# yoyololicon/spectrogram-inversion

Hardware: AMD Instinct MI355X
Metric: Griffin-Lim iterations*frames/sec at n_fft=2048 hop=512 (higher is better)
Workload: dtype f32; 1 GPU; C2: griffin_lim B64/GPU n_fft=2048 hop=512 T=1024 it=100 alpha=0.3 hann center reflect tol=0 eva_iter=10; global_batch=64, parallelism=batch-sharded x1, RCCL gather, step=phase_init + ISTFT + iterations + gather, kernel=k_fused4_td

## Files before the change

### spectrogram_inversion_amd/csrc/kernels_fast_td.h

```cpp
#pragma once
#include "fast_core.h"

namespace specinv {
namespace fast {


template <bool FIRST, typename A, typename B>
__device__ __forceinline__ const auto& td_pick(const A& a, const B& b) {
  if constexpr (FIRST) return a;
  else return b;
}


template <int R, int OV>
__device__ __forceinline__ void td_load_block(const float* __restrict__ xrow, const float* __restrict__ tailrow, long long L,
                                              int T, int c, int t_begin, int t_end, int j, int lane, int pad_mode,
                                              v2f (&q)[R / OV]) {
  if constexpr (OV == 4) load_block4<R>(xrow, tailrow, L, T, c, t_begin, t_end, j, lane, pad_mode, q);
  else load_block<R, OV>(xrow, tailrow, L, T, c, t_begin, t_end, j, lane, pad_mode, q);
}

template <int R, int OV, bool EARLY, bool EVAL>
__device__ __forceinline__ void fused_td_body(const FastArgs& a) {
  using G = Geo<R>;
  using O = Ovl<R, OV>;
  constexpr int H = G::H, M = G::M, QU = O::QU, HOP = O::HOP, NB = O::NB, PB = O::PB;
  extern __shared__ __attribute__((aligned(16))) char smem[];
  v2f* lds_win = reinterpret_cast<v2f*>(smem);
  v2f* lds_wins = lds_win + M;
  v2f* lds_tw1 = lds_win + 2 * M;
  const int wib = __builtin_amdgcn_readfirstlane(threadIdx.x >> 6);
  v2f* tr = lds_tw1 + (R - 1) * 64 + wib * G::TR;

  for (int i = threadIdx.x; i < M; i += blockDim.x) {
    const v2f wv = v2f{a.window[2 * i], a.window[2 * i + 1]};
    lds_win[i] = wv;
    lds_wins[i] = wv * a.inv_scale;
  }
  for (int i = threadIdx.x; i < (R - 1) * 64; i += blockDim.x) {
    const int k1 = i / 64 + 1, l = i & 63;
    lds_tw1[i] = unit(2.0f * (float)((l * k1) % M) / (float)M);
  }
  __syncthreads();

  int w = __builtin_amdgcn_readfirstlane(blockIdx.x * (blockDim.x >> 6) + wib);
  if (a.skew == 0 && w >= a.n_waves) return;
  const LaneConst<R> k = lane_consts<R>();
  const int lane = k.lane;
  const unsigned ulane = (unsigned)lane;
  int b = w / a.nchunks, c = w - b * a.nchunks;
  if (a.skew >= 0x10000) {
    const int cg = 3 * ((int)blockIdx.x * 4 + (wib & 3)) + (wib >> 2);
    b = cg / a.nchunks;
    c = cg - b * a.nchunks;
    w = cg;
  } else if (a.skew != 0 && (blockDim.x >> 6) == 8) {
    const int cg = 2 * ((int)blockIdx.x * 4 + (wib & 3)) + (wib >> 2);
    b = cg / a.nchunks;
    c = cg - b * a.nchunks;
    w = cg;
  } else if (a.skew != 0) {
    const int half = a.n_waves >> 1, second = w >= half ? 1 : 0, wl = w - second * half, pairs = a.nchunks >> 1;
    b = wl / pairs;
    c = 2 * (wl - b * pairs) + second;
    w = b * a.nchunks + c;
  }
  if (a.skew != 0 && w >= a.n_waves) return;
  const int t_begin = chunk_begin(c, a.T, a.nchunks, a.skew);
  const int t_end = chunk_begin(c + 1, a.T, a.nchunks, a.skew);
  const float* zrow = a.x_in + (long long)b * a.L;
  const float* tailrow = a.xtail_in + (long long)b * a.nchunks * NB * HOP;
  float* zorow = a.x_out + (long long)b * a.L;
  const bool write_x = a.x2_out != nullptr;
  float* xorow = a.x2_out + (long long)b * a.L;
  const float half_scale = 0.5f * a.fwd_scale;
  const float tds_raw = a.tds / half_scale;
  const float nlr = -a.coef;

  v2f acc[NB * QU];
#pragma unroll
  for (int i = 0; i < NB * QU; ++i) acc[i] = v2f{0.0f, 0.0f};
  double sd = 0.0, so = 0.0;
  constexpr bool TWLDS = EVAL && R >= 16;
  TwRegs<TWLDS ? 2 : R> twr_regs;
  if (!TWLDS) {
#pragma unroll
    for (int k1 = 1; k1 < R; ++k1) twr_regs.w[(TWLDS ? 1 : k1) - 1] = lds_tw1[(k1 - 1) * 64 + lane];
  }
  const TwLds twr_lds{lds_tw1, lane};
  const auto& twr = td_pick<TWLDS>(twr_lds, twr_regs);

  v2f xq[NB][QU], xn[QU];
#pragma unroll
  for (int q = 0; q < NB; ++q)
    td_load_block<R, OV>(zrow, tailrow, a.L, a.T, c, t_begin, t_end, t_begin + q, lane, a.pad_mode, xq[q]);
  td_load_block<R, OV>(zrow, tailrow, a.L, a.T, c, t_begin, t_end, t_begin + NB, lane, a.pad_mode, xn);

  constexpr bool ENVREG = !EVAL;
  v2f envc[ENVREG ? QU : 1];
  v2f envr[ENVREG ? QU : 1];
  if (ENVREG) {
    const v2f* e0 = reinterpret_cast<const v2f*>(a.env + (long long)(NB - PB) * HOP);
#pragma unroll
    for (int i = 0; i < QU; ++i) {
      envc[i] = e0[64u * i + ulane];
      envr[i] = env_rcp(envc[i]);
    }
  }
  constexpr bool WKREG = !EVAL;
  v2f wkr[WKREG ? H : 1];
  if (WKREG) {
#pragma unroll
    for (int j = 0; j < H; ++j) wkr[j] = pair_twiddle<R>(k.wn, j);
  }
  for (int t = t_begin; t < t_end; ++t) {
    asm volatile("" ::: "memory");
    v2f wn = k.wn;
    asm volatile("" : "+v"(wn));
    const long long fi = (long long)b * a.T + t;
    v4f mm[H / 2];
    v4f pp[EARLY ? H : 1];
    v2f pmid = v2f{0.0f, 0.0f};
    float mmid = 0.0f;
    __builtin_amdgcn_s_setprio(1);
    {
      const v4f* min_ = a.m_pairs + fi * (H / 2 * 64);
#pragma unroll
      for (int j = 0; j < H / 2; ++j) mm[j] = ld_stream(&min_[j * 64u + ulane]);
      if (lane == 0) {
        mmid = a.m_mid[fi];
        if (EARLY) pmid = a.Pmid_in[fi];
      }
    }
#define SPECINV_TD_C0_LOADS()                                                              \
    if (EARLY) {                                                                           \
      const v4f* pin_ = a.P_in + fi * (H * 64);                                            \
      _Pragma("unroll") for (int j = 0; j < H; ++j) pp[j] = ld_stream(&pin_[j * 64u + ulane]); \
    }
    if (!EVAL) SPECINV_TD_C0_LOADS();

    v2f z[R];
    if (EVAL) {
      const float* xrow = a.x2_in + (long long)b * a.L;
#pragma unroll
      for (int qq = 0; qq < OV; ++qq) {
        v2f q[QU];
        td_load_block<R, OV>(xrow, tailrow, a.L, a.T, c, t_begin, t_end, t + qq, lane, a.pad_mode, q);
#pragma unroll
        for (int i = 0; i < QU; ++i) z[qq * QU + i] = q[i] * lds_win[64 * (qq * QU + i) + lane];
      }
      fft_forward_t<R>(z, k, twr, tr);
      v2f rc[H];
#pragma unroll
      for (int m = H; m < R; ++m) {
        const v2f got = shfl2(z[m], k.partner);
        const v2f own = z[(m + 1) % R];
        rc[m - H] = v2f{lane == 0 ? own.x : got.x, lane == 0 ? own.y : got.y};
      }
      float fd = 0.0f, fo = 0.0f;
#pragma unroll
      for (int j = 0; j < H; ++j) {
        const v2f wk = pair_twiddle<R>(wn, j);
        v2f xk, xm;
        td_split<R>(z[j], rc[R - 1 - j - H], wk, half_scale, xk, xm);
        const float mk = (j & 1) ? mm[j / 2].z : mm[j / 2].x;
        const float mq = (j & 1) ? mm[j / 2].w : mm[j / 2].y;
        const float ok = fast_abs(xk), om = fast_abs(xm);
        const float dk = ok - mk, dm = om - mq;
        fd = fmaf(dk, dk, fmaf(dm, dm, fd));
        fo = fmaf(ok, ok, fmaf(om, om, fo));
      }
      if (lane == 0) {
        const float o = fast_abs(z[H] * v2f{a.fwd_scale, -a.fwd_scale});
        const float d = o - mmid;
        fd = fmaf(d, d, fd);
        fo = fmaf(o, o, fo);
      }
      sd += (double)fd;
      so += (double)fo;
      asm volatile("" ::: "memory");
      __builtin_amdgcn_sched_barrier(0);
      SPECINV_TD_C0_LOADS();
    }
#undef SPECINV_TD_C0_LOADS

    v2f zold[QU];
#pragma unroll
    for (int i = 0; i < QU; ++i) {
      zold[i] = xq[0][i];
#pragma unroll
      for (int q = 0; q < NB; ++q) z[q * QU + i] = xq[q][i] * lds_win[64 * (q * QU + i) + lane];
      z[NB * QU + i] = xn[i] * lds_win[64 * (NB * QU + i) + lane];
#pragma unroll
      for (int q = 0; q + 1 < NB; ++q) xq[q][i] = xq[q + 1][i];
      xq[NB - 1][i] = xn[i];
    }
    if (t + 1 < t_end)
      td_load_block<R, OV>(zrow, tailrow, a.L, a.T, c, t_begin, t_end, t + OV, lane, a.pad_mode, xn);
    __builtin_amdgcn_s_setprio(0);

    fft_forward_t<R>(z, k, twr, tr);

    v2f rc[H];
#pragma unroll
    for (int m = H; m < R; ++m) {
      const v2f got = shfl2(z[m], k.partner);
      const v2f own = z[(m + 1) % R];
      rc[m - H] = v2f{lane == 0 ? own.x : got.x, lane == 0 ? own.y : got.y};
    }

    v2f back[H];
    {
      v2f sk[H], sm[H], tt[H], yy[H], hh[H];
#pragma unroll
      for (int j = 0; j < H; ++j) {
        const v2f wk = WKREG ? wkr[WKREG ? j : 0] : pair_twiddle<R>(wn, j);
        td_split_raw<R>(z[j], rc[R - 1 - j - H], wk, sk[j], sm[j]);
        if (EARLY) {
          sk[j] = __builtin_elementwise_fma(v2f{pp[j].x, pp[j].y}, v2f{tds_raw, tds_raw}, sk[j]);
          sm[j] = __builtin_elementwise_fma(v2f{pp[j].z, pp[j].w}, v2f{tds_raw, tds_raw}, sm[j]);
        }
        tt[j] = v2f{ref_norm2(sk[j], 4.0f * kRefFloor), ref_norm2(sm[j], 4.0f * kRefFloor)};
      }
#pragma unroll
      for (int j = 0; j < H; ++j) yy[j] = v2f{__builtin_amdgcn_rsqf(tt[j].x), __builtin_amdgcn_rsqf(tt[j].y)};
#pragma unroll
      for (int j = 0; j < H; ++j) hh[j] = tt[j] * yy[j];
#pragma unroll
      for (int j = 0; j < H; ++j) tt[j] = __builtin_elementwise_fma(-hh[j], yy[j], v2f{1.0f, 1.0f});
#pragma unroll
      for (int j = 0; j < H; ++j) yy[j] = __builtin_elementwise_fma(yy[j] * 0.5f, tt[j], yy[j]);
#pragma unroll
      for (int j = 0; j < H; ++j) {
        const v2f mp = (j & 1) ? v2f{mm[j / 2].z, mm[j / 2].w} : v2f{mm[j / 2].x, mm[j / 2].y};
        sk[j] = scale_lo(sk[j], mp);
        sm[j] = scale_hi(sm[j], mp);
      }
#pragma unroll
      for (int j = 0; j < H; ++j) {
        const v2f wk = WKREG ? wkr[WKREG ? j : 0] : pair_twiddle<R>(wn, j);
        v2f ak = scale_lo(sk[j], yy[j]);
        v2f am = scale_hi(sm[j], yy[j]);
        if (j == 0 && lane == 0) {
          ak.y = 0.0f;
          am.y = 0.0f;
        }
        const v2f e2i = add_conj(ak, am);
        const v2f o2i = cmulc(sub_conj(ak, am), wk);
        z[j] = add_i(e2i, o2i);
        back[j] = conj_sub_i(e2i, o2i);
      }
    }
    v2f zmid;
    {
      v2f smid = z[H] * v2f{a.fwd_scale, -a.fwd_scale};
      if (EARLY) smid = v2f{fmaf(a.tds, pmid.x, smid.x), fmaf(a.tds, pmid.y, smid.y)};
      const v2f am = (smid * mmid) * ref_rcp_abs(ref_norm2(smid));
      zmid = am * v2f{2.0f, -2.0f};
    }
#pragma unroll
    for (int m = H; m < R; ++m) {
      const v2f got = shfl2(back[R - 1 - m], k.partner);
      const v2f l0 = (m == H) ? zmid : back[(R - m) % H];
      z[m] = v2f{lane == 0 ? l0.x : got.x, lane == 0 ? l0.y : got.y};
    }

    fft_inverse_t<R>(z, k, twr, tr);

#pragma unroll
    for (int u = 0; u < R; ++u) z[u] = z[u] * lds_wins[64 * u + lane];
    if (t >= PB) {
      const long long o0 = (long long)(t - PB) * HOP;
      const v2f* envp = reinterpret_cast<const v2f*>(a.env + o0);
      v2f* xo = reinterpret_cast<v2f*>(xorow + o0);
      v2f* zo = reinterpret_cast<v2f*>(zorow + o0);
      v2f ev[QU], er[QU];
      if (!ENVREG) {
#pragma unroll
        for (int i = 0; i < QU; ++i) {
          ev[i] = envp[64u * i + ulane];
          er[i] = env_rcp(ev[i]);
        }
      } else if (t >= NB) {
#pragma unroll
        for (int i = 0; i < QU; ++i) {
          ev[i] = envc[ENVREG ? i : 0];
          er[i] = envr[ENVREG ? i : 0];
        }
      } else {
#pragma unroll
        for (int i = 0; i < QU; ++i) ev[i] = envp[64u * i + ulane];
#pragma unroll
        for (int i = 0; i < QU; ++i) asm volatile("" : "+v"(ev[i]));
#pragma unroll
        for (int i = 0; i < QU; ++i) er[i] = env_rcp(ev[i]);
      }
#pragma unroll
      for (int i = 0; i < QU; ++i) {
        const v2f xv = env_apply_r(acc[i] + z[i], ev[i], er[i]);
        const v2f zv = v2f{fmaf(nlr, zold[i].x, xv.x), fmaf(nlr, zold[i].y, xv.y)};
        if (write_x) xo[64u * i + ulane] = xv;
        zo[64u * i + ulane] = zv;
      }
    }
#pragma unroll
    for (int i = 0; i < QU; ++i) {
#pragma unroll
      for (int q = 0; q + 1 < NB; ++q) acc[q * QU + i] = acc[(q + 1) * QU + i] + z[(q + 1) * QU + i];
      acc[(NB - 1) * QU + i] = z[NB * QU + i];
    }
  }
  if (t_end == a.T) {
#pragma unroll
    for (int q = 0; q < PB - 1; ++q) {
      const long long o0 = (long long)(a.T + q - PB) * HOP;
      const v2f* envp = reinterpret_cast<const v2f*>(a.env + o0);
      v2f* xo = reinterpret_cast<v2f*>(xorow + o0);
      v2f* zo = reinterpret_cast<v2f*>(zorow + o0);
#pragma unroll
      for (int i = 0; i < QU; ++i) {
        const v2f xv = env_apply(acc[q * QU + i], envp[64u * i + ulane]);
        if (write_x) xo[64u * i + ulane] = xv;
        zo[64u * i + ulane] = v2f{fmaf(nlr, xq[q][i].x, xv.x), fmaf(nlr, xq[q][i].y, xv.y)};
      }
    }
  } else {
    v2f* tl = reinterpret_cast<v2f*>(a.xtail_out + ((long long)b * a.nchunks + c) * NB * HOP);
#pragma unroll
    for (int q = 0; q < NB; ++q) {
      const v2f* envp = reinterpret_cast<const v2f*>(a.env + (long long)(t_end + q - PB) * HOP);
#pragma unroll
      for (int i = 0; i < QU; ++i) tl[(q * QU + i) * 64u + ulane] = env_apply(acc[q * QU + i], envp[64u * i + ulane]);
    }
  }
  if (EVAL) {
    const double d = wave_sum(sd), o = wave_sum(so);
    if (lane == 0) {
      a.partials[2 * (long long)w] = d;
      a.partials[2 * (long long)w + 1] = o;
    }
  }
}

template <int R, bool EARLY, bool EVAL>
__global__ __launch_bounds__(R == 8 ? 768 : 64 * kFused4Waves, R == 8 ? kR8Waves : kMinWaves) void k_fused4_td(FastArgs a) {
  fused_td_body<R, 4, EARLY, EVAL>(a);
}
template <int R, int OV, bool EARLY, bool EVAL>
__global__ __launch_bounds__(256, R >= 32 ? 1 : R == 8 ? kR8Waves : kMinWaves) void k_fused_td(FastArgs a) {
  fused_td_body<R, OV, EARLY, EVAL>(a);
}

constexpr int kEvalSub = kEvalPieces;
template <int R, int OV>
__global__ __launch_bounds__(256, kEvalWaves) void k_eval_td(FastArgs a) {
  using G = Geo<R>;
  using O = Ovl<R, OV>;
  constexpr int H = G::H, M = G::M, QU = O::QU, HOP = O::HOP, NB = O::NB;
  extern __shared__ __attribute__((aligned(16))) char smem[];
  v2f* lds_win = reinterpret_cast<v2f*>(smem);
  v2f* lds_tw1 = lds_win + M;
  const int wib = __builtin_amdgcn_readfirstlane(threadIdx.x >> 6);
  v2f* tr = lds_tw1 + (R - 1) * 64 + wib * G::TR;
  for (int i = threadIdx.x; i < M; i += blockDim.x) lds_win[i] = v2f{a.window[2 * i], a.window[2 * i + 1]};
  for (int i = threadIdx.x; i < (R - 1) * 64; i += blockDim.x) {
    const int k1 = i / 64 + 1, l = i & 63;
    lds_tw1[i] = unit(2.0f * (float)((l * k1) % M) / (float)M);
  }
  __syncthreads();
  const int w = __builtin_amdgcn_readfirstlane(blockIdx.x * 4 + wib);
  if (w >= a.n_waves * kEvalSub) return;
  const LaneConst<R> k = lane_consts<R>();
  const int lane = k.lane;
  const unsigned ulane = (unsigned)lane;
  const int cw = w / kEvalSub, sub = w - cw * kEvalSub;
  const int b = cw / a.nchunks, c = cw - b * a.nchunks;
  const int t_begin = chunk_begin(c, a.T, a.nchunks, a.skew), t_end = chunk_begin(c + 1, a.T, a.nchunks, a.skew);
  const int s_begin = t_begin + (sub * (t_end - t_begin)) / kEvalSub, s_end = t_begin + ((sub + 1) * (t_end - t_begin)) / kEvalSub;
  const float* xrow = a.x2_in + (long long)b * a.L;
  const float* tailrow = a.xtail_in + (long long)b * a.nchunks * NB * HOP;
  const float half_scale = 0.5f * a.fwd_scale;
  TwRegs<R> twr;
#pragma unroll
  for (int k1 = 1; k1 < R; ++k1) twr.w[k1 - 1] = lds_tw1[(k1 - 1) * 64 + lane];
  double sd = 0.0, so = 0.0;
  v2f xq[NB][QU], xn[QU];
#pragma unroll
  for (int q = 0; q < NB; ++q)
    td_load_block<R, OV>(xrow, tailrow, a.L, a.T, c, t_begin, t_end, s_begin + q, lane, a.pad_mode, xq[q]);
  td_load_block<R, OV>(xrow, tailrow, a.L, a.T, c, t_begin, t_end, s_begin + NB, lane, a.pad_mode, xn);
  for (int t = s_begin; t < s_end; ++t) {
    asm volatile("" ::: "memory");
    v2f wn = k.wn;
    asm volatile("" : "+v"(wn));
    const long long fi = (long long)b * a.T + t;
    v4f mm[H / 2];
    float mmid = 0.0f;
    {
      const v4f* min_ = a.m_pairs + fi * (H / 2 * 64);
#pragma unroll
      for (int j = 0; j < H / 2; ++j) mm[j] = ld_stream(&min_[j * 64u + ulane]);
      if (lane == 0) mmid = a.m_mid[fi];
    }
    v2f z[R];
#pragma unroll
    for (int i = 0; i < QU; ++i) {
#pragma unroll
      for (int q = 0; q < NB; ++q) z[q * QU + i] = xq[q][i] * lds_win[64 * (q * QU + i) + lane];
      z[NB * QU + i] = xn[i] * lds_win[64 * (NB * QU + i) + lane];
#pragma unroll
      for (int q = 0; q + 1 < NB; ++q) xq[q][i] = xq[q + 1][i];
      xq[NB - 1][i] = xn[i];
    }
    if (t + 1 < s_end) td_load_block<R, OV>(xrow, tailrow, a.L, a.T, c, t_begin, t_end, t + OV, lane, a.pad_mode, xn);
    fft_forward_t<R>(z, k, twr, tr);
    v2f rc[H];
#pragma unroll
    for (int m = H; m < R; ++m) {
      const v2f got = shfl2(z[m], k.partner);
      const v2f own = z[(m + 1) % R];
      rc[m - H] = v2f{lane == 0 ? own.x : got.x, lane == 0 ? own.y : got.y};
    }
    float fd = 0.0f, fo = 0.0f;
#pragma unroll
    for (int j = 0; j < H; ++j) {
      const v2f wk = pair_twiddle<R>(wn, j);
      v2f xk, xm;
      td_split<R>(z[j], rc[R - 1 - j - H], wk, half_scale, xk, xm);
      const float mk = (j & 1) ? mm[j / 2].z : mm[j / 2].x;
      const float mq = (j & 1) ? mm[j / 2].w : mm[j / 2].y;
      const float ok = fast_abs(xk), om = fast_abs(xm);
      const float dk = ok - mk, dm = om - mq;
      fd = fmaf(dk, dk, fmaf(dm, dm, fd));
      fo = fmaf(ok, ok, fmaf(om, om, fo));
    }
    if (lane == 0) {
      const float o = fast_abs(z[H] * v2f{a.fwd_scale, -a.fwd_scale});
      const float d = o - mmid;
      fd = fmaf(d, d, fd);
      fo = fmaf(o, o, fo);
    }
    sd += (double)fd;
    so += (double)fo;
  }
  const double d = wave_sum(sd), o = wave_sum(so);
  if (lane == 0) {
    a.partials[2 * (long long)w] = d;
    a.partials[2 * (long long)w + 1] = o;
  }
}

}
}
```

Before: 320.3 million iterations*frames/s.

## Add specialized radix-16 TD FFT path with LDS transpose and streamline envelope handling

Adds a hand-specialized R==16 forward/inverse FFT built from explicit DFT16 stages with constant-folded twiddles, a cross-lane DFT4, and an LDS transpose through precomputed scratch pointers. The fused and eval TD kernels now call it in place of the generic fft_forward_t/fft_inverse_t. The change also reuses the env register arrays instead of copying them, applies the window multiply only to the overlap part and defers the last block's scaling into the accumulator update, and marks xn as undefined on the last iteration to avoid keeping it live. The aim is fewer ALU and shuffle operations and less register pressure in the inner frame loop. In exchange it brings an R-specific code path and more complex LDS indexing.

```diff
diff --git a/spectrogram_inversion_amd/csrc/kernels_fast_td.h b/spectrogram_inversion_amd/csrc/kernels_fast_td.h
--- a/spectrogram_inversion_amd/csrc/kernels_fast_td.h
+++ b/spectrogram_inversion_amd/csrc/kernels_fast_td.h
@@ -18,6 +18,107 @@
                                               v2f (&q)[R / OV]) {
   if constexpr (OV == 4) load_block4<R>(xrow, tailrow, L, T, c, t_begin, t_end, j, lane, pad_mode, q);
   else load_block<R, OV>(xrow, tailrow, L, T, c, t_begin, t_end, j, lane, pad_mode, q);
+}
+
+using lds_v2f = __attribute__((address_space(3))) v2f;
+struct TdScratch {
+  volatile lds_v2f* q;
+  lds_v2f* b;
+};
+template <int R>
+__device__ __forceinline__ TdScratch td_scratch(v2f* tr, const LaneConst<R>& k) {
+  TdScratch s;
+  s.q = (volatile lds_v2f*)(tr + k.tr_q);
+  s.b = (lds_v2f*)(tr + k.tr_b);
+  asm volatile("" : "+v"(s.b));
+  return s;
+}
+
+template <bool INV>
+__device__ __forceinline__ void dft4_rot2(v2f& a0, v2f& a1, v2f& a2, v2f& a3) {
+  const v2f t0 = INV ? add_i(a0, a2) : sub_i(a0, a2);
+  const v2f t1 = INV ? sub_i(a0, a2) : add_i(a0, a2);
+  const v2f t2 = a1 + a3, d = a1 - a3;
+  a0 = t0 + t2;
+  a2 = t0 - t2;
+  a1 = INV ? add_i(t1, d) : sub_i(t1, d);
+  a3 = INV ? sub_i(t1, d) : add_i(t1, d);
+}
+template <bool INV>
+__device__ __forceinline__ void td_dft16(v2f (&a)[16]) {
+  constexpr float c1 = 0.92387953251128675613f, s1 = 0.38268343236508977173f, h = 0.70710678118654752440f;
+#pragma unroll
+  for (int n0 = 0; n0 < 4; ++n0) dft4<INV>(a[n0], a[n0 + 4], a[n0 + 8], a[n0 + 12]);
+  dirmul_x4<INV, true>(a[5], a[6], a[7], a[9], v2f{c1, -s1}, v2f{h, -h}, v2f{s1, -c1}, v2f{h, -h});
+  dirmul_x4<INV, true>(a[11], a[13], a[14], a[15], v2f{-h, -h}, v2f{s1, -c1}, v2f{-h, -h}, v2f{-c1, s1});
+  dft4<INV>(a[0], a[1], a[2], a[3]);
+  dft4<INV>(a[4], a[5], a[6], a[7]);
+  dft4_rot2<INV>(a[8], a[9], a[10], a[11]);
+  dft4<INV>(a[12], a[13], a[14], a[15]);
+  v2f o[16];
+#pragma unroll
+  for (int k0 = 0; k0 < 4; ++k0)
+#pragma unroll
+    for (int k1 = 0; k1 < 4; ++k1) o[k1 + 4 * k0] = a[k0 + 4 * k1];
+#pragma unroll
+  for (int i = 0; i < 16; ++i) a[i] = o[i];
+}
+
+template <int R, typename TW>
+__device__ __forceinline__ void td_fft_forward(v2f (&z)[R], const LaneConst<R>& k, const TW& tw, v2f* __restrict__ tr,
+                                               const TdScratch& sc) {
+  if constexpr (R == 16) {
+    td_dft16<false>(z);
+    cmul_all<R, true, false, 1>(z, tw);
+#pragma unroll
+    for (int g = 0; g < R; g += 4) xlane_dft4_in<false>(z[g], z[g + 1], z[g + 2], z[g + 3]);
+#pragma unroll
+    for (int g = 0; g < R; g += 4) {
+      z[g + 2] = cmul(z[g + 2], k.postq[0]);
+      z[g + 1] = cmul(z[g + 1], k.postq[1]);
+      z[g + 3] = cmul(z[g + 3], k.postq[2]);
+    }
+#pragma unroll
+    for (int g = 0; g < R; g += 4) {
+      sc.q[(0 * R + g) * (R + 1)] = z[g];
+      sc.q[(1 * R + g) * (R + 1)] = z[g + 2];
+      sc.q[(2 * R + g) * (R + 1)] = z[g + 1];
+      sc.q[(3 * R + g) * (R + 1)] = z[g + 3];
+    }
+#pragma unroll
+    for (int i = 0; i < R; ++i) z[i] = sc.b[i];
+    td_dft16<false>(z);
+  } else {
+    fft_forward_t<R>(z, k, tw, tr);
+  }
+}
+template <int R, typename TW>
+__device__ __forceinline__ void td_fft_inverse(v2f (&z)[R], const LaneConst<R>& k, const TW& tw, v2f* __restrict__ tr,
+                                               const TdScratch& sc) {
+  if constexpr (R == 16) {
+    td_dft16<true>(z);
+#pragma unroll
+    for (int i = 0; i < R; ++i) sc.b[i] = z[i];
+#pragma unroll
+    for (int g = 0; g < R; g += 4) {
+      z[g] = sc.q[(0 * R + g) * (R + 1)];
+      z[g + 2] = sc.q[(1 * R + g) * (R + 1)];
+      z[g + 1] = sc.q[(2 * R + g) * (R + 1)];
+      z[g + 3] = sc.q[(3 * R + g) * (R + 1)];
+    }
+#pragma unroll
+    for (int g = 0; g < R; g += 4) {
+      z[g + 2] = cmulc(z[g + 2], k.postq[0]);
+      z[g + 1] = cmulc(z[g + 1], k.postq[1]);
+      z[g + 3] = cmulc(z[g + 3], k.postq[2]);
+    }
+#pragma unroll
+    for (int g = 0; g < R; g += 4) xlane_dft4_out<true>(z[g], z[g + 1], z[g + 2], z[g + 3]);
+    cmul_all<R, true, true, 1>(z, tw);
+    td_dft16<true>(z);
+  } else {
+    fft_inverse_t<R>(z, k, tw, tr);
+  }
 }
 
 template <int R, int OV, bool EARLY, bool EVAL>
@@ -46,6 +147,7 @@
   int w = __builtin_amdgcn_readfirstlane(blockIdx.x * (blockDim.x >> 6) + wib);
   if (a.skew == 0 && w >= a.n_waves) return;
   const LaneConst<R> k = lane_consts<R>();
+  const TdScratch tsc = td_scratch<R>(tr, k);
   const int lane = k.lane;
   const unsigned ulane = (unsigned)lane;
   int b = w / a.nchunks, c = w - b * a.nchunks;
@@ -97,8 +199,7 @@
   td_load_block<R, OV>(zrow, tailrow, a.L, a.T, c, t_begin, t_end, t_begin + NB, lane, a.pad_mode, xn);
 
   constexpr bool ENVREG = !EVAL;
-  v2f envc[ENVREG ? QU : 1];
-  v2f envr[ENVREG ? QU : 1];
+  v2f envc[QU], envr[QU];
   if (ENVREG) {
     const v2f* e0 = reinterpret_cast<const v2f*>(a.env + (long long)(NB - PB) * HOP);
 #pragma unroll
@@ -116,7 +217,7 @@
   for (int t = t_begin; t < t_end; ++t) {
     asm volatile("" ::: "memory");
     v2f wn = k.wn;
-    asm volatile("" : "+v"(wn));
+    if (!WKREG) asm volatile("" : "+v"(wn));
     const long long fi = (long long)b * a.T + t;
     v4f mm[H / 2];
     v4f pp[EARLY ? H : 1];
@@ -149,7 +250,7 @@
 #pragma unroll
         for (int i = 0; i < QU; ++i) z[qq * QU + i] = q[i] * lds_win[64 * (qq * QU + i) + lane];
       }
-      fft_forward_t<R>(z, k, twr, tr);
+      td_fft_forward<R>(z, k, twr, tr, tsc);
       v2f rc[H];
 #pragma unroll
       for (int m = H; m < R; ++m) {
@@ -195,11 +296,15 @@
       for (int q = 0; q + 1 < NB; ++q) xq[q][i] = xq[q + 1][i];
       xq[NB - 1][i] = xn[i];
     }
-    if (t + 1 < t_end)
+    if (t + 1 < t_end) {
       td_load_block<R, OV>(zrow, tailrow, a.L, a.T, c, t_begin, t_end, t + OV, lane, a.pad_mode, xn);
+    } else {
+#pragma unroll
+      for (int i = 0; i < QU; ++i) asm volatile("" : "=v"(xn[i]));
+    }
     __builtin_amdgcn_s_setprio(0);
 
-    fft_forward_t<R>(z, k, twr, tr);
+    td_fft_forward<R>(z, k, twr, tr, tsc);
 
     v2f rc[H];
 #pragma unroll
@@ -265,40 +370,33 @@
       z[m] = v2f{lane == 0 ? l0.x : got.x, lane == 0 ? l0.y : got.y};
     }
 
-    fft_inverse_t<R>(z, k, twr, tr);
-
-#pragma unroll
-    for (int u = 0; u < R; ++u) z[u] = z[u] * lds_wins[64 * u + lane];
+    td_fft_inverse<R>(z, k, twr, tr, tsc);
+
+#pragma unroll
+    for (int u = 0; u < NB * QU; ++u) z[u] = z[u] * lds_wins[64 * u + lane];
     if (t >= PB) {
       const long long o0 = (long long)(t - PB) * HOP;
       const v2f* envp = reinterpret_cast<const v2f*>(a.env + o0);
       v2f* xo = reinterpret_cast<v2f*>(xorow + o0);
       v2f* zo = reinterpret_cast<v2f*>(zorow + o0);
-      v2f ev[QU], er[QU];
       if (!ENVREG) {
 #pragma unroll
         for (int i = 0; i < QU; ++i) {
-          ev[i] = envp[64u * i + ulane];
-          er[i] = env_rcp(ev[i]);
+          envc[i] = envp[64u * i + ulane];
+          envr[i] = env_rcp(envc[i]);
         }
-      } else if (t >= NB) {
-#pragma unroll
-        for (int i = 0; i < QU; ++i) {
-          ev[i] = envc[ENVREG ? i : 0];
-          er[i] = envr[ENVREG ? i : 0];
-        }
-      } else {
-#pragma unroll
-        for (int i = 0; i < QU; ++i) ev[i] = envp[64u * i + ulane];
-#pragma unroll
-        for (int i = 0; i < QU; ++i) asm volatile("" : "+v"(ev[i]));
-#pragma unroll
-        for (int i = 0; i < QU; ++i) er[i] = env_rcp(ev[i]);
+      } else if (t <= NB) {
+#pragma unroll
+        for (int i = 0; i < QU; ++i) envc[i] = envp[64u * i + ulane];
+#pragma unroll
+        for (int i = 0; i < QU; ++i) asm volatile("" : "+v"(envc[i]));
+#pragma unroll
+        for (int i = 0; i < QU; ++i) envr[i] = env_rcp(envc[i]);
       }
 #pragma unroll
       for (int i = 0; i < QU; ++i) {
-        const v2f xv = env_apply_r(acc[i] + z[i], ev[i], er[i]);
-        const v2f zv = v2f{fmaf(nlr, zold[i].x, xv.x), fmaf(nlr, zold[i].y, xv.y)};
+        const v2f xv = env_apply_r(acc[i] + z[i], envc[i], envr[i]);
+        const v2f zv = __builtin_elementwise_fma(v2f{nlr, nlr}, zold[i], xv);
         if (write_x) xo[64u * i + ulane] = xv;
         zo[64u * i + ulane] = zv;
       }
@@ -307,8 +405,9 @@
     for (int i = 0; i < QU; ++i) {
 #pragma unroll
       for (int q = 0; q + 1 < NB; ++q) acc[q * QU + i] = acc[(q + 1) * QU + i] + z[(q + 1) * QU + i];
-      acc[(NB - 1) * QU + i] = z[NB * QU + i];
-    }
+    }
+#pragma unroll
+    for (int i = 0; i < QU; ++i) acc[(NB - 1) * QU + i] = z[NB * QU + i] * lds_wins[64 * (NB * QU + i) + lane];
   }
   if (t_end == a.T) {
 #pragma unroll
@@ -371,6 +470,7 @@
   const int w = __builtin_amdgcn_readfirstlane(blockIdx.x * 4 + wib);
   if (w >= a.n_waves * kEvalSub) return;
   const LaneConst<R> k = lane_consts<R>();
+  const TdScratch tsc = td_scratch<R>(tr, k);
   const int lane = k.lane;
   const unsigned ulane = (unsigned)lane;
   const int cw = w / kEvalSub, sub = w - cw * kEvalSub;
@@ -412,8 +512,13 @@
       for (int q = 0; q + 1 < NB; ++q) xq[q][i] = xq[q + 1][i];
       xq[NB - 1][i] = xn[i];
     }
-    if (t + 1 < s_end) td_load_block<R, OV>(xrow, tailrow, a.L, a.T, c, t_begin, t_end, t + OV, lane, a.pad_mode, xn);
-    fft_forward_t<R>(z, k, twr, tr);
+    if (t + 1 < s_end) {
+      td_load_block<R, OV>(xrow, tailrow, a.L, a.T, c, t_begin, t_end, t + OV, lane, a.pad_mode, xn);
+    } else {
+#pragma unroll
+      for (int i = 0; i < QU; ++i) asm volatile("" : "=v"(xn[i]));
+    }
+    td_fft_forward<R>(z, k, twr, tr, tsc);
     v2f rc[H];
 #pragma unroll
     for (int m = H; m < R; ++m) {
```

After: 325.9 million iterations*frames/s (median of 6 runs). +1.8%, better.
